# VITA-Group/FasterSeg

Hardware: NVIDIA H100
Metric: fasterseg_student_fps_1024x2048 (higher is better)
Workload: dtype fp16

## Files before the change

fasterseg_b200/csrc/conv_tc.cu:

```cuda
#include "fsb_common.cuh"
#include "fsb_internal.h"

namespace fsb {

constexpr int kTileM = 128;
constexpr int kMaxStages = 8;
constexpr int kThreads = 256;
constexpr int kAccLd = kTileM + 4;

struct ConvTcParams {
  CUtensorMap tmap_a[4];
  CUtensorMap tmap_b;
  CUtensorMap tmap_y[2];
  int tma_store;
  int tail_w;
  int taps;
  int tap_map[9];
  int tap_dh[9];
  int tap_dw[9];
  int tap_widx[9];
  int k_chunks;
  int Ho, Wo;
  int tiles_w, tiles_h;
  int tw, th;
  int win_pitch, win_rows;
  int win_sbo;
  int win_half;
  int win_stride;
  int m_half, m_grp;
  int Cout;
  int stages;
  int y_cstride;
  uint32_t flags;
  const float* scale;
  const float* shift;
  __half* y;
  float* stats;
  int stats_C;
  int stats_off;
};

template <int NT>
__host__ __device__ constexpr uint32_t conv_tc_out_bytes() { return static_cast<uint32_t>((NT + 63) / 64) * kTileM * 128; }
template <int NT>
__host__ __device__ constexpr uint32_t conv_tc_epilogue_bytes() { return conv_tc_out_bytes<NT>() + static_cast<uint32_t>(NT) * kAccLd * 4; }


template <int BK, int NT, bool WIN>
__global__ void __launch_bounds__(kThreads, NT <= 64 ? 2 : 1)
conv_tc_kernel(const __grid_constant__ ConvTcParams p) {
  extern __shared__ uint8_t smem_raw[];
  __shared__ __align__(8) uint64_t full_bar[kMaxStages];
  __shared__ __align__(8) uint64_t empty_bar[kMaxStages];
  __shared__ __align__(8) uint64_t win_full[2];
  __shared__ __align__(8) uint64_t win_empty[2];
  __shared__ float s_scale[NT];
  __shared__ float s_shift[NT];

  pdl_launch_dependents();
  const int warp = threadIdx.x >> 5;
  const int lane = threadIdx.x & 31;
  constexpr uint32_t kABytes = kTileM * BK * 2;
  constexpr uint32_t kStageBytes = WIN ? NT * BK * 2 : kABytes + NT * BK * 2;
  static_assert(!WIN || BK == 64, "windows are 128B-swizzled 64-channel rows");
  uint8_t* smem = reinterpret_cast<uint8_t*>((reinterpret_cast<uintptr_t>(smem_raw) + 1023) & ~uintptr_t(1023));

  int t = blockIdx.x;
  const int tile_w = t % p.tiles_w;
  t /= p.tiles_w;
  const int tile_h = t % p.tiles_h;
  const int img = t / p.tiles_h;
  const int w0 = tile_w * p.tw;
  const int h0 = tile_h * p.th;
  const int n0 = blockIdx.y * NT;
  const int k_iters = p.taps * p.k_chunks;

  if (warp == 0 && lane == 0) {
    tma_prefetch_desc(&p.tmap_a[0]);
    tma_prefetch_desc(&p.tmap_b);
    for (int s = 0; s < p.stages; ++s) {
      mbar_init(&full_bar[s], 1);
      mbar_init(&empty_bar[s], 4);
    }
    for (int w = 0; w < 2; ++w) {
      mbar_init(&win_full[w], 1);
      mbar_init(&win_empty[w], 4);
    }
    mbar_fence_init();
  }
  pdl_wait();
  for (int c = threadIdx.x; c < NT; c += kThreads) {
    const int ch = n0 + c;
    const bool ok = ch < p.Cout;
    s_scale[c] = (ok && (p.flags & FSB_CONV_AFFINE) && p.scale) ? p.scale[ch] : 1.0f;
    s_shift[c] = (ok && (p.flags & FSB_CONV_AFFINE) && p.shift) ? p.shift[ch] : 0.0f;
  }
  __syncthreads();

// ... 2 lines not shown
    const uint32_t win_bytes = static_cast<uint32_t>(p.win_rows * p.win_pitch) * 128u;
    RingPos rp, rw;
    for (int kc = 0; kc < p.k_chunks; ++kc) {
      mbar_wait_inline(&win_empty[rw.s], rw.phase ^ 1u);
      if (elect_one()) {
        mbar_arrive_expect_tx(&win_full[rw.s], win_bytes);
        tma_load_4d(smem + rw.s * p.win_stride, &p.tmap_a[0], &win_full[rw.s], kc * BK, w0 + p.tap_dw[0], h0 + p.tap_dh[0], img);
      }
      __syncwarp();
      rw.advance(2);
      for (int tap = 0; tap < 9; ++tap) {
        mbar_wait_inline(&empty_bar[rp.s], rp.phase ^ 1u);
        if (elect_one()) {
          mbar_arrive_expect_tx(&full_bar[rp.s], kStageBytes);
          tma_load_3d(bring + rp.s * kStageBytes, &p.tmap_b, &full_bar[rp.s], kc * BK, n0, tap);
        }
        __syncwarp();
        rp.advance(p.stages);
      }
    }
  } else if (warp == 0) {
    RingPos rp;
    uint8_t* sa = smem;
    for (int tap = 0; tap < p.taps; ++tap) {
      const CUtensorMap* ma = &p.tmap_a[p.tap_map[tap]];
      const int cw = w0 + p.tap_dw[tap];
      const int chh = h0 + p.tap_dh[tap];
      const int wi = p.tap_widx[tap];
      for (int kc = 0; kc < p.k_chunks; ++kc) {
        mbar_wait_inline(&empty_bar[rp.s], rp.phase ^ 1u);
        if (elect_one()) {
          mbar_arrive_expect_tx(&full_bar[rp.s], kStageBytes);
          tma_load_4d(sa, ma, &full_bar[rp.s], kc * BK, cw, chh, img);
          tma_load_3d(sa + kABytes, &p.tmap_b, &full_bar[rp.s], kc * BK, n0, wi);
        }
        __syncwarp();
        sa += kStageBytes;
        rp.advance(p.stages);
        if (rp.s == 0) sa = smem;
      }
    }
  } else if (warp >= 4) {
    const int tw = threadIdx.x - 128;
    float acc[2][NT / 2];
#pragma unroll
    for (int h = 0; h < 2; ++h)
#pragma unroll
      for (int i = 0; i < NT / 2; ++i) acc[h][i] = 0.f;
    const uint32_t sa0 = smem_u32(smem);
    const uint64_t da0 = wgmma_desc_kmajor(sa0, BK * 2);
    const uint64_t db0 = wgmma_desc_kmajor(sa0 + kABytes, BK * 2);
    constexpr uint32_t kHalf = (64 * BK * 2) >> 4;
    if constexpr (WIN) {
      const uint64_t dw0 = wgmma_desc(sa0, 16, p.win_sbo, 128);
      const uint64_t dbr = wgmma_desc_kmajor(sa0 + 2 * p.win_stride, 128);
      const uint64_t whalf = static_cast<uint64_t>(p.win_half * 8);
      RingPos rp, rw;
      int prev = -1, prev_w = -1;
      for (int kc = 0; kc < p.k_chunks; ++kc) {
        mbar_wait_inline(&win_full[rw.s], rw.phase);
        const uint64_t dwin = dw0 + static_cast<uint64_t>(rw.s * (p.win_stride >> 4));
        for (int tap = 0; tap < 9; ++tap) {
// ... 1 lines not shown
          mbar_wait_inline(&full_bar[rp.s], rp.phase);
          wgmma_fence();
          const uint64_t da = dwin + static_cast<uint64_t>((r * p.win_pitch + sx) * 8);
          const uint64_t db = dbr + static_cast<uint64_t>(rp.s * (kStageBytes >> 4));
#pragma unroll
          for (int k = 0; k < BK / 16; ++k) {
            wgmma_f16<NT, 0>(acc[0], da + static_cast<uint64_t>(2 * k), db + static_cast<uint64_t>(2 * k));
            wgmma_f16<NT, 0>(acc[1], da + whalf + static_cast<uint64_t>(2 * k), db + static_cast<uint64_t>(2 * k));
          }
          wgmma_commit();
          wgmma_wait<1>();
          if (prev >= 0 && lane == 0) mbar_arrive(&empty_bar[prev]);
          if (tap == 0 && prev_w >= 0 && lane == 0) mbar_arrive(&win_empty[prev_w]);
          prev = rp.s;
          rp.advance(p.stages);
        }
        prev_w = rw.s;
        rw.advance(2);
      }
    } else {
    RingPos rp;
    uint32_t doff = 0;
    int prev = -1;
    for (int it = 0; it < k_iters; ++it) {
      mbar_wait_inline(&full_bar[rp.s], rp.phase);
      wgmma_fence();
#pragma unroll
      for (int k = 0; k < BK / 16; ++k) {
        const uint64_t da = da0 + doff + static_cast<uint64_t>(2 * k), db = db0 + doff + static_cast<uint64_t>(2 * k);
        wgmma_f16<NT, 0>(acc[0], da, db);
        wgmma_f16<NT, 0>(acc[1], da + kHalf, db);
      }
      wgmma_commit();
      wgmma_wait<1>();
      if (prev >= 0 && lane == 0) mbar_arrive(&empty_bar[prev]);
      prev = rp.s;
      doff += kStageBytes >> 4;
      rp.advance(p.stages);
      if (rp.s == 0) doff = 0;
    }
    }
    wgmma_wait<0>();
    float* s_acc = reinterpret_cast<float*>(smem + conv_tc_out_bytes<NT>());
    named_bar_sync(1, 128);
    if constexpr (WIN) {
      const int row0 = wgmma_row(tw, 0);
      const int m0 = (row0 >> 3) * p.m_grp + (row0 & 7);
#pragma unroll
      for (int h = 0; h < 2; ++h) {
        float* s_h = s_acc + h * p.m_half + m0;
#pragma unroll
        for (int i = 0; i < NT / 2; ++i) s_h[wgmma_col(tw, i) * kAccLd + ((i >> 1) & 1) * p.m_grp] = acc[h][i];
      }
    } else {
#pragma unroll
      for (int h = 0; h < 2; ++h)
#pragma unroll
        for (int i = 0; i < NT / 2; ++i) s_acc[wgmma_col(tw, i) * kAccLd + 64 * h + wgmma_row(tw, i)] = acc[h][i];
    }
    named_bar_sync(1, 128);

    const int q = warp & 3;
    const int m = q * 32 + lane;
    const int oh = h0 + m / p.tw;
    const int ow = w0 + m % p.tw;
    const bool pix_ok = (oh < p.Ho) && (ow < p.Wo);
    __half* yrow = p.y + (static_cast<size_t>(img) * p.Ho * p.Wo + static_cast<size_t>(oh) * p.Wo + ow) * p.y_cstride + n0;
    const bool out_f32 = (p.flags & FSB_CONV_OUT_F32) != 0;
    float* yrow32 = reinterpret_cast<float*>(p.y) +
                    (static_cast<size_t>(img) * p.Ho * p.Wo + static_cast<size_t>(oh) * p.Wo + ow) * p.y_cstride + n0;
    const bool vec_ok = out_f32 ? ((reinterpret_cast<uintptr_t>(yrow32) & 15) == 0) : ((reinterpret_cast<uintptr_t>(yrow) & 15) == 0);
    const bool relu = (p.flags & FSB_CONV_RELU) != 0;
    const bool do_stats = (p.flags & FSB_CONV_STATS) != 0 && p.stats != nullptr;
    float* s_stat = reinterpret_cast<float*>(smem);
    for (int c0 = 0; c0 < NT; c0 += 64) {
      const int nb = min(4, (NT - c0) >> 4);
#pragma unroll
      for (int b = 0; b < 4; ++b) {
      if (b >= nb) break;
      const int c = c0 + 16 * b;
      float f[16];
#pragma unroll
      for (int j = 0; j < 16; ++j) f[j] = s_acc[(c + j) * kAccLd + m];
      if (do_stats) {
#pragma unroll
        for (int j = 0; j < 16; ++j) {
          float a = pix_ok ? f[j] : 0.f;
          float b = a * a;
#pragma unroll
          for (int o = 16; o > 0; o >>= 1) {
            a += __shfl_xor_sync(0xffffffffu, a, o);
            b += __shfl_xor_sync(0xffffffffu, b, o);
          }
          if (lane == 0) {
            s_stat[(q * 2 + 0) * NT + c + j] = a;
            s_stat[(q * 2 + 1) * NT + c + j] = b;
          }
        }
      }
#pragma unroll
      for (int j = 0; j < 16; ++j) {
        float x = f[j] * s_scale[c + j] + s_shift[c + j];
        f[j] = relu ? fmaxf(x, 0.f) : x;
      }
      if (pix_ok && out_f32) {
        const int remaining = p.Cout - (n0 + c);
        if (remaining >= 16 && vec_ok) {
          float4* dst = reinterpret_cast<float4*>(yrow32 + c);
          dst[0] = make_float4(f[0], f[1], f[2], f[3]);
          dst[1] = make_float4(f[4], f[5], f[6], f[7]);
          dst[2] = make_float4(f[8], f[9], f[10], f[11]);
          dst[3] = make_float4(f[12], f[13], f[14], f[15]);
        } else {
#pragma unroll
          for (int j = 0; j < 16; ++j)
            if (j < remaining) yrow32[c + j] = f[j];
        }
      } else if (p.tma_store) {
        uint4 o0, o1;
        o0.x = pack_half2(f[0], f[1]);
        o0.y = pack_half2(f[2], f[3]);
        o0.z = pack_half2(f[4], f[5]);
        o0.w = pack_half2(f[6], f[7]);
        o1.x = pack_half2(f[8], f[9]);
        o1.y = pack_half2(f[10], f[11]);
        o1.z = pack_half2(f[12], f[13]);
        o1.w = pack_half2(f[14], f[15]);
        uint8_t* slab = smem + static_cast<size_t>(c0 >> 6) * (kTileM * 128);
        const int ch16 = (c - c0) >> 3;
        if (NT - c0 >= 64) {
          *reinterpret_cast<uint4*>(slab + m * 128 + ((ch16 ^ (m & 7)) << 4)) = o0;
          *reinterpret_cast<uint4*>(slab + m * 128 + (((ch16 + 1) ^ (m & 7)) << 4)) = o1;
        } else {
          uint8_t* row = slab + m * (p.tail_w * 2) + (ch16 << 4);
          *reinterpret_cast<uint4*>(row) = o0;
          *reinterpret_cast<uint4*>(row + 16) = o1;
        }
      } else if (pix_ok) {
        const int remaining = p.Cout - (n0 + c);
        if (remaining >= 16 && vec_ok) {
          uint4 o0, o1;
          o0.x = pack_half2(f[0], f[1]);
          o0.y = pack_half2(f[2], f[3]);
          o0.z = pack_half2(f[4], f[5]);
          o0.w = pack_half2(f[6], f[7]);
          o1.x = pack_half2(f[8], f[9]);
          o1.y = pack_half2(f[10], f[11]);
          o1.z = pack_half2(f[12], f[13]);
          o1.w = pack_half2(f[14], f[15]);
          uint4* dst = reinterpret_cast<uint4*>(yrow + c);
          dst[0] = o0;
          dst[1] = o1;
        } else {
#pragma unroll
          for (int j = 0; j < 16; ++j)
            if (j < remaining) yrow[c + j] = __float2half_rn(f[j]);
        }
      }
      }
      if (p.tma_store) {
        fence_proxy_async_smem();
        named_bar_sync(1, 128);
        if (warp == 4 && lane == 0) {
          const bool full = (NT - c0) >= 64;
          tma_store_4d(&p.tmap_y[full ? 0 : 1], smem + static_cast<size_t>(c0 >> 6) * (kTileM * 128), n0 + c0, w0, h0, img);
          tma_store_commit();
        }
      }
    }
    if (p.tma_store && warp == 4 && lane == 0) tma_store_wait_read();
    if (do_stats) {
      named_bar_sync(2, 128);
      float* row = p.stats + static_cast<size_t>(blockIdx.x) * 2 * p.stats_C + p.stats_off;
      for (int ch = static_cast<int>(threadIdx.x) - 128; ch < NT; ch += 128) {
        if (n0 + ch >= p.Cout) continue;
        float a = s_stat[0 * NT + ch], b = s_stat[1 * NT + ch];
#pragma unroll
        for (int w = 1; w < 4; ++w) {
          a += s_stat[(w * 2 + 0) * NT + ch];
          b += s_stat[(w * 2 + 1) * NT + ch];
        }
        row[n0 + ch] = a;
        row[p.stats_C + n0 + ch] = b;
      }
    }
  }
  __syncthreads();
}

static int encode_tiled(CUtensorMap* map, const void* base, int rank, const uint64_t* dims, const uint64_t* strides_bytes,
                        const uint32_t* box, int swizzle_bytes) {
  PFN_encodeTiled enc = get_encode_tiled();
  if (!enc) return set_error(FSB_ERR_CUDA, "cuTensorMapEncodeTiled entry point unavailable");
  cuuint32_t estr[5] = {1, 1, 1, 1, 1};
  cuuint64_t gdim[5];
  cuuint64_t gstr[5];
  cuuint32_t bdim[5];
  for (int i = 0; i < rank; ++i) {
    gdim[i] = dims[i];
    bdim[i] = box[i];
  }
  for (int i = 0; i + 1 < rank; ++i) gstr[i] = strides_bytes[i];
  CUtensorMapSwizzle sw = swizzle_bytes == 128 ? CU_TENSOR_MAP_SWIZZLE_128B
                          : (swizzle_bytes == 64 ? CU_TENSOR_MAP_SWIZZLE_64B
                                                 : (swizzle_bytes == 32 ? CU_TENSOR_MAP_SWIZZLE_32B : CU_TENSOR_MAP_SWIZZLE_NONE));
  CUresult r = enc(map, CU_TENSOR_MAP_DATA_TYPE_FLOAT16, static_cast<cuuint32_t>(rank), const_cast<void*>(base), gdim, gstr,
                   bdim, estr, CU_TENSOR_MAP_INTERLEAVE_NONE, sw, CU_TENSOR_MAP_L2_PROMOTION_L2_256B,
                   CU_TENSOR_MAP_FLOAT_OOB_FILL_NONE);
  if (r != CUDA_SUCCESS) {
    char buf[256];
// ... 25 lines not shown

enum ConvTcMode { kPerTap, kWindow, kStrip };
static ConvTcMode conv_tc_mode(const fsb_conv_desc* d) {
  if (d->ksize != 3 || d->stride != 1 || d->dil != 1) return kPerTap;
  const int o = opt(OPT_CONV_TC2);
  if (o == 0) return kPerTap;
  if (o == 2 && d->Cin % 64 == 0 && !(d->flags & FSB_CONV_STATS)) return kStrip;
  return kWindow;
}
bool conv_tc_strip(const fsb_conv_desc* d) { return conv_tc_mode(d) == kStrip; }

int conv_tc_m_tiles(const fsb_conv_desc* d) {
  if (conv_tc_strip(d)) return ((d->Wo + kTileM - 1) / kTileM) * d->Ho * d->N;
  const int tw = d->Wo >= 16 ? 16 : 8, th = kTileM / tw;
  return ((d->Wo + tw - 1) / tw) * ((d->Ho + th - 1) / th) * d->N;
}

int conv_tc_supported(const fsb_conv_desc* d) {
  if (d->Cin < 16 || (d->x_cstride % 8) != 0) return 0;
  if (!(d->ksize == 1 || d->ksize == 3) || !(d->stride == 1 || d->stride == 2)) return 0;
  return 1;
}

template <int BK, int NT, bool WIN = false>
static int conv_tc_run(dim3 grid, size_t smem_bytes, cudaStream_t stream, const ConvTcParams& p) {
  if (int rc = ensure_dyn_smem(reinterpret_cast<const void*>(conv_tc_kernel<BK, NT, WIN>), 220 * 1024, "cudaFuncSetAttribute(conv_tc)"))
    return rc;
  const cudaError_t e = launch_kernel(conv_tc_kernel<BK, NT, WIN>, grid, dim3(kThreads), smem_bytes, stream, p);
  return e == cudaSuccess ? FSB_OK : set_cuda_error(e, "conv_tc launch");
}

template <int BK, bool WIN>
static int conv_tc_run_nt(int n_tile, dim3 grid, size_t smem_bytes, cudaStream_t stream, const ConvTcParams& p) {
  switch (n_tile) {
    case 16: return conv_tc_run<BK, 16, WIN>(grid, smem_bytes, stream, p);
    case 32: return conv_tc_run<BK, 32, WIN>(grid, smem_bytes, stream, p);
    case 48: return conv_tc_run<BK, 48, WIN>(grid, smem_bytes, stream, p);
    case 64: return conv_tc_run<BK, 64, WIN>(grid, smem_bytes, stream, p);
    case 96: return conv_tc_run<BK, 96, WIN>(grid, smem_bytes, stream, p);
    default: return conv_tc_run<BK, 128, WIN>(grid, smem_bytes, stream, p);
  }
}

int conv_tc_launch(const fsb_conv_desc* d, const void* x, const void* wpacked, const float* scale, const float* shift,
                   void* y, float* stats, cudaStream_t stream, const ConvTcCustom* cu, bool window_ok) {
  const ConvGeom g = conv_geom(d);
  if (cu && (d->stride != 1 || (d->flags & (FSB_CONV_OUT_F32 | FSB_CONV_STATS))))
    return set_error(FSB_ERR_INVALID, "conv_tc: custom tap tables need a stride-1 fp16 problem");
  if ((reinterpret_cast<uintptr_t>(x) & 15) || (reinterpret_cast<uintptr_t>(wpacked) & 15))
    return set_error(FSB_ERR_INVALID, "conv_tc: x / wpacked must be 16-byte aligned");
  ConvTcParams p;
  memset(&p, 0, sizeof(p));
  const ConvTcMode mode = cu ? kPerTap : conv_tc_mode(d);
  const bool strip = mode == kStrip;
  p.taps = cu ? cu->ntaps : g.taps;
  p.Ho = cu ? cu->Ho : d->Ho;
  p.Wo = cu ? cu->Wo : d->Wo;
  p.tw = strip ? kTileM : (p.Wo >= 16 ? 16 : 8);
  p.th = kTileM / p.tw;
  p.tiles_w = (p.Wo + p.tw - 1) / p.tw;
  p.tiles_h = (p.Ho + p.th - 1) / p.th;
  for (int i = 0; i < 9; ++i) p.tap_widx[i] = i;
  p.Cout = d->Cout;
  static const int kNt[] = {16, 32, 48, 64, 96, 128};
  const int m_tiles = p.tiles_w * p.tiles_h * d->N;
  int n_tiles = (g.npad + 127) / 128;
  int ni = 0;
  while (kNt[ni] * n_tiles < g.npad) ++ni;
  int n_tile = kNt[ni];
  n_tiles = (g.npad + n_tile - 1) / n_tile;
  const int sms = sm_count();
  const int nt_min = opt(OPT_CONV_NTILE_MIN) >= 16 ? opt(OPT_CONV_NTILE_MIN) : 32;
  while (m_tiles * n_tiles < sms && ni > 0 && kNt[ni - 1] >= nt_min) {
    n_tile = kNt[--ni];
    n_tiles = (g.npad + n_tile - 1) / n_tile;
  }
  const bool win = strip || (mode == kWindow && ((window_ok && m_tiles * n_tiles > sms && !(d->flags & FSB_CONV_STATS)) ||
                                                 opt(OPT_CONV_TC2) == 1));
  const int bk = win ? 64 : g.bk;
  p.k_chunks = (g.kpad + bk - 1) / bk;
  if (win) {
    p.win_pitch = p.tw + 2;
    p.win_rows = p.th + 2;
    p.win_stride = (p.win_rows * p.win_pitch * 128 + 1023) / 1024 * 1024;
    p.m_half = 64;
    p.m_grp = 8;
    if (strip) {
      p.win_sbo = 8 * 128;
      p.win_half = 64;
    } else if (p.tw == 16) {
      p.win_sbo = p.win_pitch * 128;
      p.win_half = 8;
      p.m_half = 8;
      p.m_grp = 16;
    } else {
      p.win_sbo = p.win_pitch * 128;
      p.win_half = 8 * p.win_pitch;
    }
  }
  p.y_cstride = d->y_cstride;
  p.flags = d->flags;
  p.scale = scale;
  p.shift = shift;
  p.y = static_cast<__half*>(y);
  p.stats = stats;
  p.stats_C = d->stats_C > 0 ? d->stats_C : d->Cout;
  p.stats_off = d->stats_off;
  if ((d->flags & FSB_CONV_STATS) && stats && (d->stats_off < 0 || d->stats_off + d->Cout > p.stats_C))
    return set_error(FSB_ERR_INVALID, "conv_tc: stats_off + Cout exceeds stats_C");

  const size_t stage_bytes = (win ? 0 : static_cast<size_t>(kTileM) * bk * 2) + static_cast<size_t>(n_tile) * bk * 2;
  const int k_iters = p.taps * p.k_chunks;
  const size_t smem_budget = (n_tile == 128 || m_tiles * n_tiles <= sms || strip) ? 200 * 1024 : 100 * 1024;
  const size_t win_bytes = win ? 2 * static_cast<size_t>(p.win_stride) : 0;
  int stages = static_cast<int>((smem_budget - win_bytes) / stage_bytes);
  if (stages < 2) stages = 2;
  if (stages > kMaxStages) stages = kMaxStages;
  if (stages > k_iters) stages = k_iters;
  p.stages = stages;
  const size_t epi_bytes = n_tile == 16 ? conv_tc_epilogue_bytes<16>() : n_tile == 32 ? conv_tc_epilogue_bytes<32>()
                           : n_tile == 48 ? conv_tc_epilogue_bytes<48>() : n_tile == 64 ? conv_tc_epilogue_bytes<64>()
                           : n_tile == 96 ? conv_tc_epilogue_bytes<96>() : conv_tc_epilogue_bytes<128>();
  size_t smem_bytes = (win_bytes + stage_bytes * stages > epi_bytes ? win_bytes + stage_bytes * stages : epi_bytes) + 1024;
  p.tma_store = 0;
  if (!(d->flags & (FSB_CONV_OUT_F32 | FSB_CONV_STATS)) && d->Cout % 8 == 0 && d->y_cstride % 8 == 0 && (reinterpret_cast<uintptr_t>(y) & 15) == 0 &&
      n_tile % 8 == 0 && (cu || opt(OPT_NO_TMA_STORE) <= 0)) {
    const uint64_t ycs = static_cast<uint64_t>(d->y_cstride) * 2;
    uint64_t dims[4] = {static_cast<uint64_t>(d->Cout), static_cast<uint64_t>(d->Wo), static_cast<uint64_t>(d->Ho),
                        static_cast<uint64_t>(d->N)};
    uint64_t str[3] = {ycs, ycs * d->Wo, ycs * d->Wo * d->Ho};
    if (cu) {
      y = const_cast<void*>(cu->y_base);
      for (int i = 0; i < 4; ++i) dims[i] = cu->y_dims[i];
      for (int i = 0; i < 3; ++i) str[i] = cu->y_strides[i];
    }
    const uint32_t box64[4] = {64u, static_cast<uint32_t>(p.tw), static_cast<uint32_t>(p.th), 1u};
    int rc = 0;
    if (n_tile >= 64) rc = encode_tiled(&p.tmap_y[0], y, 4, dims, str, box64, 128);
    p.tail_w = n_tile % 64;
    if (!rc && p.tail_w) {
      const uint32_t boxt[4] = {static_cast<uint32_t>(p.tail_w), static_cast<uint32_t>(p.tw), static_cast<uint32_t>(p.th), 1u};
      rc = encode_tiled(&p.tmap_y[1], y, 4, dims, str, boxt, 0);
    }
    if (rc) return rc;
    if (n_tile < 64) p.tmap_y[0] = p.tmap_y[1];
    p.tma_store = 1;
  }
  if (cu && !p.tma_store) return set_error(FSB_ERR_UNSUPPORTED, "conv_tc: custom output lattice needs the TMA-store epilogue");
// ... 36 lines not shown
        used[ph * 2 + pw] = true;
      }
    for (int ph = 0; ph < 2; ++ph)
      for (int pw = 0; pw < 2; ++pw) {
        if (!used[ph * 2 + pw]) continue;
        const int Hp = (d->H - ph + 1) / 2, Wp = (d->W - pw + 1) / 2;
        if (Hp <= 0 || Wp <= 0) return set_error(FSB_ERR_INVALID, "conv_tc: empty parity plane");
        const uint64_t dims[4] = {static_cast<uint64_t>(d->Cin), static_cast<uint64_t>(Wp), static_cast<uint64_t>(Hp),
                                  static_cast<uint64_t>(d->N)};
        const uint64_t str[3] = {2 * cs, 2 * cs * d->W, cs * d->W * d->H};
        const __half* base = xb + (static_cast<size_t>(ph) * d->W + pw) * d->x_cstride;
        int rc = encode_tiled(&p.tmap_a[ph * 2 + pw], base, 4, dims, str, boxA, g.bk * 2);
        if (rc) return rc;
      }
    if (!used[0]) p.tmap_a[0] = p.tmap_a[p.tap_map[0]];
  }
  {
    const uint64_t dims[3] = {static_cast<uint64_t>(g.kpad), static_cast<uint64_t>(g.npad), static_cast<uint64_t>(g.taps)};
    const uint64_t str[2] = {static_cast<uint64_t>(g.kpad) * 2, static_cast<uint64_t>(g.kpad) * g.npad * 2};
    const uint32_t boxB[3] = {static_cast<uint32_t>(bk), static_cast<uint32_t>(n_tile), 1u};
    int rc = encode_tiled(&p.tmap_b, wpacked, 3, dims, str, boxB, bk * 2);
    if (rc) return rc;
  }
  const dim3 grid(static_cast<unsigned>(m_tiles), static_cast<unsigned>(n_tiles));
  if (win) return conv_tc_run_nt<64, true>(n_tile, grid, smem_bytes, stream, p);
  if (g.bk == 64) return conv_tc_run_nt<64, false>(n_tile, grid, smem_bytes, stream, p);
  return conv_tc_run_nt<32, false>(n_tile, grid, smem_bytes, stream, p);
}

}
```

fasterseg_b200/csrc/fsb_common.cuh:

```cuda
#pragma once
#include <cuda.h>
#include <cuda_fp16.h>
#include <cuda_runtime.h>
#include <stdint.h>
#include <stdio.h>

namespace fsb {

__device__ __forceinline__ uint32_t smem_u32(const void* p) {
  return static_cast<uint32_t>(__cvta_generic_to_shared(p));
}
__device__ __forceinline__ bool elect_one() {
  uint32_t pred = 0;
  asm volatile(
      "{\n\t.reg .pred P;\n\telect.sync _|P, 0xffffffff;\n\tselp.u32 %0, 1, 0, P;\n\t}\n"
      : "=r"(pred));
  return pred != 0;
}

__device__ __forceinline__ void pdl_launch_dependents() { asm volatile("griddepcontrol.launch_dependents;" ::: "memory"); }
__device__ __forceinline__ void pdl_wait() { asm volatile("griddepcontrol.wait;" ::: "memory"); }

__device__ __forceinline__ void mbar_init(uint64_t* bar, uint32_t count) {
  asm volatile("mbarrier.init.shared::cta.b64 [%0], %1;" ::"r"(smem_u32(bar)), "r"(count) : "memory");
// ... 73 lines not shown
__device__ __forceinline__ void tma_store_4d(const CUtensorMap* m, const void* smem_src, int c0, int c1, int c2, int c3) {
  asm volatile("cp.async.bulk.tensor.4d.global.shared::cta.bulk_group [%0, {%2, %3, %4, %5}], [%1];"
               ::"l"(reinterpret_cast<uint64_t>(m)), "r"(smem_u32(smem_src)), "r"(c0), "r"(c1), "r"(c2), "r"(c3)
               : "memory");
}
__device__ __forceinline__ void tma_store_commit() { asm volatile("cp.async.bulk.commit_group;" ::: "memory"); }
__device__ __forceinline__ void tma_store_wait_read() { asm volatile("cp.async.bulk.wait_group.read 0;" ::: "memory"); }
__device__ __forceinline__ void fence_proxy_async_smem() { asm volatile("fence.proxy.async.shared::cta;" ::: "memory"); }
__device__ __forceinline__ void named_bar_sync(int id, int nthreads) {
  asm volatile("bar.sync %0, %1;" ::"r"(id), "r"(nthreads) : "memory");
}

__device__ __forceinline__ void cluster_sync_all_threads() {
  asm volatile("barrier.cluster.arrive.release.aligned;\n\tbarrier.cluster.wait.acquire.aligned;" ::: "memory");
}
__device__ __forceinline__ uint32_t mapa_cluster(uint32_t cta_smem_addr, uint32_t target_rank) {
  uint32_t r;
  asm volatile("mapa.shared::cluster.u32 %0, %1, %2;" : "=r"(r) : "r"(cta_smem_addr), "r"(target_rank));
  return r;
}
__device__ __forceinline__ void st_cluster_u32(uint32_t cluster_addr, uint32_t v) {
  asm volatile("st.shared::cluster.u32 [%0], %1;" ::"r"(cluster_addr), "r"(v) : "memory");
}

__device__ __forceinline__ void wgmma_fence() { asm volatile("wgmma.fence.sync.aligned;" ::: "memory"); }
__device__ __forceinline__ void wgmma_commit() { asm volatile("wgmma.commit_group.sync.aligned;" ::: "memory"); }
template <int N>
__device__ __forceinline__ void wgmma_wait() { asm volatile("wgmma.wait_group.sync.aligned %0;" ::"n"(N) : "memory"); }
__device__ __forceinline__ int wgmma_row(int t, int i) { return 16 * (t >> 5) + ((t & 31) >> 2) + 8 * ((i >> 1) & 1); }
__device__ __forceinline__ int wgmma_col(int t, int i) { return 8 * (i >> 2) + 2 * (t & 3) + (i & 1); }

template <int TR>
__device__ __forceinline__ void wgmma_m64n16k16(float (&d)[8], uint64_t da, uint64_t db) {
  asm volatile(
      "wgmma.mma_async.sync.aligned.m64n16k16.f32.f16.f16 "
      "{%0, %1, %2, %3, %4, %5, %6, %7}, %8, %9, 1, 1, 1, %10, %11;"
      : "+f"(d[0]), "+f"(d[1]), "+f"(d[2]), "+f"(d[3]), "+f"(d[4]), "+f"(d[5]), "+f"(d[6]), "+f"(d[7])
      : "l"(da), "l"(db), "n"(TR), "n"(TR));
}
template <int TR>
__device__ __forceinline__ void wgmma_m64n32k16(float (&d)[16], uint64_t da, uint64_t db) {
  asm volatile(
      "wgmma.mma_async.sync.aligned.m64n32k16.f32.f16.f16 "
      "{%0, %1, %2, %3, %4, %5, %6, %7, %8, %9, %10, %11, %12, %13, %14, %15}, %16, %17, 1, 1, 1, %18, %19;"
      : "+f"(d[0]), "+f"(d[1]), "+f"(d[2]), "+f"(d[3]), "+f"(d[4]), "+f"(d[5]), "+f"(d[6]), "+f"(d[7]), "+f"(d[8]), "+f"(d[9]), "+f"(d[10]), "+f"(d[11]), "+f"(d[12]), "+f"(d[13]), "+f"(d[14]), "+f"(d[15])
      : "l"(da), "l"(db), "n"(TR), "n"(TR));
// ... 65 lines not shown
```

fasterseg_b200/csrc/fsb_internal.h:

```cpp
#pragma once
#include <cuda.h>
#include <cuda_runtime.h>
#include <stdint.h>
#include <stdio.h>
#include <stdlib.h>
#include <string.h>

#include "../../include/fsb200.h"

namespace fsb {

int set_error(int code, const char* msg);
int set_cuda_error(cudaError_t e, const char* where);

typedef CUresult (*PFN_encodeTiled)(CUtensorMap*, CUtensorMapDataType, cuuint32_t, void*, const cuuint64_t*,
                                    const cuuint64_t*, const cuuint32_t*, const cuuint32_t*, CUtensorMapInterleave,
                                    CUtensorMapSwizzle, CUtensorMapL2promotion, CUtensorMapFloatOOBfill);
PFN_encodeTiled get_encode_tiled();

struct ConvGeom {
  int taps;
  int bk;
  int kpad;
  int npad;
// ... 7 lines not shown
  OPT_CONV_TC2 = 0,
  OPT_TC2_R,
  OPT_TC2_ASTAGES,
  OPT_NO_TMA_STORE,
  OPT_DGRAD_S2_DIRECT,
  OPT_WGRAD_TC,
  OPT_CONV_PERSIST,
  OPT_PERSIST_OCC,
  OPT_PERSIST_STAGES,
  OPT_UPSAMPLE_V2,
  OPT_DETERMINISTIC,
  OPT_CONV_TC3,
  OPT_CONV_TC4,
  OPT_CONV_TC5,
  OPT_CONV_KSPLIT,
  OPT_CONV_NTILE_MIN,
  OPT_COUNT
};
int opt(Opt o);

int ensure_dyn_smem(const void* kernel, int bytes, const char* what);

template <typename... KArgs, typename... Args>
inline cudaError_t launch_kernel(void (*kernel)(KArgs...), dim3 grid, dim3 block, size_t smem, cudaStream_t stream,
                                 Args&&... args) {
  cudaLaunchConfig_t cfg;
  memset(&cfg, 0, sizeof(cfg));
  cfg.gridDim = grid;
  cfg.blockDim = block;
  cfg.dynamicSmemBytes = smem;
  cfg.stream = stream;
  cudaLaunchAttribute attr[1];
  attr[0].id = cudaLaunchAttributeProgrammaticStreamSerialization;
  attr[0].val.programmaticStreamSerializationAllowed = 1;
  cfg.attrs = attr;
  cfg.numAttrs = pdl_enabled() ? 1 : 0;
  return cudaLaunchKernelEx(&cfg, kernel, static_cast<KArgs>(args)...);
}

extern thread_local cudaError_t g_launch_err;
#define FSB_LAUNCH(kernel, grid, block, smem, stream, ...) \
  (::fsb::g_launch_err = ::fsb::launch_kernel(kernel, grid, block, smem, stream, __VA_ARGS__))
inline cudaError_t last_launch_error() {
  cudaError_t e = g_launch_err;
  g_launch_err = cudaSuccess;
  if (e == cudaSuccess) e = cudaGetLastError();
  return e;
}

struct ConvTcCustom {
  int ntaps;
  int dh[9], dw[9], widx[9];
  int Ho, Wo;
  const void* y_base;
  uint64_t y_dims[4];
  uint64_t y_strides[3];
};
int conv_tc_supported(const fsb_conv_desc* d);
bool conv_tc_strip(const fsb_conv_desc* d);
int conv_tc_launch(const fsb_conv_desc* d, const void* x, const void* wpacked, const float* scale, const float* shift,
                   void* y, float* stats, cudaStream_t stream, const ConvTcCustom* cu = nullptr, bool window_ok = true);
int conv_wgrad_tc_supported(const fsb_conv_desc* d, int dy_cstride);
int conv_wgrad_tc_launch(const fsb_conv_desc* d, const void* x, const void* dy, int dcs, float* dw, int64_t so, int64_t si,
                         float gscale, cudaStream_t stream);
int conv_direct_launch(const fsb_conv_desc* d, const void* x, const void* wpacked, const float* scale, const float* shift,
// ... 4 lines not shown
```

fasterseg_b200/csrc/wgrad_tc.cu:

```cuda
#include "fsb_common.cuh"
#include "fsb_internal.h"

namespace fsb {

constexpr int kWgThreads = 256;
constexpr int kWgMaxStages = 6;
constexpr int kWgPix = 128;
constexpr int kWgSub = kWgPix * 128;

struct WgradTcParams {
  CUtensorMap tmap_dy;
  CUtensorMap tmap_x[4];
  int taps, ksize;
  int tap_map[9], tap_dh[9], tap_dw[9];
  int tiles_w, tiles_h, n_img;
  int tw, th;
  int Cout, Cin;
  int co_tiles, ci_tiles;
  int chunks;
  int stages;
  float inv_gscale;
  float* dw;
  long long so, si;
};
// ... 191 lines not shown
        const int ph = ((qh % 2) + 2) % 2, pw = ((qw % 2) + 2) % 2;
        p.tap_map[tp] = ph * 2 + pw;
        p.tap_dh[tp] = floordiv2(qh);
        p.tap_dw[tp] = floordiv2(qw);
        used[ph * 2 + pw] = true;
      }
    for (int ph = 0; ph < 2; ++ph)
      for (int pw = 0; pw < 2; ++pw) {
        if (!used[ph * 2 + pw]) continue;
        const int Hp = (d->H - ph + 1) / 2, Wp = (d->W - pw + 1) / 2;
        if (Hp <= 0 || Wp <= 0) return set_error(FSB_ERR_INVALID, "wgrad_tc: empty parity plane");
        const uint64_t dims[4] = {static_cast<uint64_t>(d->Cin), static_cast<uint64_t>(Wp), static_cast<uint64_t>(Hp),
                                  static_cast<uint64_t>(d->N)};
        const uint64_t str[3] = {2 * cs, 2 * cs * d->W, cs * d->W * d->H};
        int rc = encode_tiled_generic(&p.tmap_x[ph * 2 + pw], xb + (static_cast<size_t>(ph) * d->W + pw) * d->x_cstride, 4, dims,
                                      str, box, 128);
        if (rc) return rc;
      }
  }
  const void* kernel = ci_tile == 128 ? reinterpret_cast<const void*>(conv_wgrad_tc_kernel<128>)
                                      : reinterpret_cast<const void*>(conv_wgrad_tc_kernel<64>);
  if (int rc = ensure_dyn_smem(kernel, 220 * 1024, "cudaFuncSetAttribute(conv_wgrad_tc)")) return rc;
  dim3 grid(static_cast<unsigned>(fixed), static_cast<unsigned>(chunks));
  const cudaError_t e = ci_tile == 128 ? launch_kernel(conv_wgrad_tc_kernel<128>, grid, dim3(kWgThreads), smem_bytes, stream, p)
                                       : launch_kernel(conv_wgrad_tc_kernel<64>, grid, dim3(kWgThreads), smem_bytes, stream, p);
  if (e != cudaSuccess) return set_cuda_error(e, "conv_wgrad_tc launch");
  return FSB_OK;
}

}
```

Baseline: 2136.

## Add cluster-based split-K for tensor-core conv with DSMEM reduction

```diff
diff --git a/fasterseg_b200/csrc/conv_tc.cu b/fasterseg_b200/csrc/conv_tc.cu
--- a/fasterseg_b200/csrc/conv_tc.cu
+++ b/fasterseg_b200/csrc/conv_tc.cu
@@ -46,7 +46,7 @@
 __host__ __device__ constexpr uint32_t conv_tc_epilogue_bytes() { return conv_tc_out_bytes<NT>() + static_cast<uint32_t>(NT) * kAccLd * 4; }
 
 
-template <int BK, int NT, bool WIN>
+template <int BK, int NT, bool WIN, bool SPLIT>
 __global__ void __launch_bounds__(kThreads, NT <= 64 ? 2 : 1)
 conv_tc_kernel(const __grid_constant__ ConvTcParams p) {
   extern __shared__ uint8_t smem_raw[];
@@ -63,6 +63,7 @@
   constexpr uint32_t kABytes = kTileM * BK * 2;
   constexpr uint32_t kStageBytes = WIN ? NT * BK * 2 : kABytes + NT * BK * 2;
   static_assert(!WIN || BK == 64, "windows are 128B-swizzled 64-channel rows");
+  static_assert(!(WIN && SPLIT), "the K split runs on the per-tap mode only");
   uint8_t* smem = reinterpret_cast<uint8_t*>((reinterpret_cast<uintptr_t>(smem_raw) + 1023) & ~uintptr_t(1023));
 
   int t = blockIdx.x;
@@ -74,6 +75,8 @@
   const int h0 = tile_h * p.th;
   const int n0 = blockIdx.y * NT;
   const int k_iters = p.taps * p.k_chunks;
+  const int it_begin = SPLIT ? static_cast<int>(blockIdx.z) * k_iters / static_cast<int>(gridDim.z) : 0;
+  const int it_end = SPLIT ? static_cast<int>(blockIdx.z + 1) * k_iters / static_cast<int>(gridDim.z) : k_iters;
 
   if (warp == 0 && lane == 0) {
     tma_prefetch_desc(&p.tmap_a[0]);
@@ -122,22 +125,21 @@
   } else if (warp == 0) {
     RingPos rp;
     uint8_t* sa = smem;
-    for (int tap = 0; tap < p.taps; ++tap) {
-      const CUtensorMap* ma = &p.tmap_a[p.tap_map[tap]];
-      const int cw = w0 + p.tap_dw[tap];
-      const int chh = h0 + p.tap_dh[tap];
-      const int wi = p.tap_widx[tap];
-      for (int kc = 0; kc < p.k_chunks; ++kc) {
-        mbar_wait_inline(&empty_bar[rp.s], rp.phase ^ 1u);
-        if (elect_one()) {
-          mbar_arrive_expect_tx(&full_bar[rp.s], kStageBytes);
-          tma_load_4d(sa, ma, &full_bar[rp.s], kc * BK, cw, chh, img);
-          tma_load_3d(sa + kABytes, &p.tmap_b, &full_bar[rp.s], kc * BK, n0, wi);
-        }
-        __syncwarp();
-        sa += kStageBytes;
-        rp.advance(p.stages);
-        if (rp.s == 0) sa = smem;
+    int tap = it_begin / p.k_chunks, kc = it_begin - tap * p.k_chunks;
+    for (int it = it_begin; it < it_end; ++it) {
+      mbar_wait_inline(&empty_bar[rp.s], rp.phase ^ 1u);
+      if (elect_one()) {
+        mbar_arrive_expect_tx(&full_bar[rp.s], kStageBytes);
+        tma_load_4d(sa, &p.tmap_a[p.tap_map[tap]], &full_bar[rp.s], kc * BK, w0 + p.tap_dw[tap], h0 + p.tap_dh[tap], img);
+        tma_load_3d(sa + kABytes, &p.tmap_b, &full_bar[rp.s], kc * BK, n0, p.tap_widx[tap]);
+      }
+      __syncwarp();
+      sa += kStageBytes;
+      rp.advance(p.stages);
+      if (rp.s == 0) sa = smem;
+      if (++kc == p.k_chunks) {
+        kc = 0;
+        ++tap;
       }
     }
   } else if (warp >= 4) {
@@ -185,7 +187,7 @@
     RingPos rp;
     uint32_t doff = 0;
     int prev = -1;
-    for (int it = 0; it < k_iters; ++it) {
+    for (int it = it_begin; it < it_end; ++it) {
       mbar_wait_inline(&full_bar[rp.s], rp.phase);
       wgmma_fence();
 #pragma unroll
@@ -223,85 +225,64 @@
     }
     named_bar_sync(1, 128);
 
-    const int q = warp & 3;
-    const int m = q * 32 + lane;
-    const int oh = h0 + m / p.tw;
-    const int ow = w0 + m % p.tw;
-    const bool pix_ok = (oh < p.Ho) && (ow < p.Wo);
-    __half* yrow = p.y + (static_cast<size_t>(img) * p.Ho * p.Wo + static_cast<size_t>(oh) * p.Wo + ow) * p.y_cstride + n0;
-    const bool out_f32 = (p.flags & FSB_CONV_OUT_F32) != 0;
-    float* yrow32 = reinterpret_cast<float*>(p.y) +
-                    (static_cast<size_t>(img) * p.Ho * p.Wo + static_cast<size_t>(oh) * p.Wo + ow) * p.y_cstride + n0;
-    const bool vec_ok = out_f32 ? ((reinterpret_cast<uintptr_t>(yrow32) & 15) == 0) : ((reinterpret_cast<uintptr_t>(yrow) & 15) == 0);
-    const bool relu = (p.flags & FSB_CONV_RELU) != 0;
-    const bool do_stats = (p.flags & FSB_CONV_STATS) != 0 && p.stats != nullptr;
-    float* s_stat = reinterpret_cast<float*>(smem);
-    for (int c0 = 0; c0 < NT; c0 += 64) {
-      const int nb = min(4, (NT - c0) >> 4);
-#pragma unroll
-      for (int b = 0; b < 4; ++b) {
-      if (b >= nb) break;
-      const int c = c0 + 16 * b;
-      float f[16];
-#pragma unroll
-      for (int j = 0; j < 16; ++j) f[j] = s_acc[(c + j) * kAccLd + m];
-      if (do_stats) {
+    if constexpr (!SPLIT) {
+      const int q = warp & 3;
+      const int m = q * 32 + lane;
+      const int oh = h0 + m / p.tw;
+      const int ow = w0 + m % p.tw;
+      const bool pix_ok = (oh < p.Ho) && (ow < p.Wo);
+      __half* yrow = p.y + (static_cast<size_t>(img) * p.Ho * p.Wo + static_cast<size_t>(oh) * p.Wo + ow) * p.y_cstride + n0;
+      const bool out_f32 = (p.flags & FSB_CONV_OUT_F32) != 0;
+      float* yrow32 = reinterpret_cast<float*>(p.y) +
+                      (static_cast<size_t>(img) * p.Ho * p.Wo + static_cast<size_t>(oh) * p.Wo + ow) * p.y_cstride + n0;
+      const bool vec_ok = out_f32 ? ((reinterpret_cast<uintptr_t>(yrow32) & 15) == 0) : ((reinterpret_cast<uintptr_t>(yrow) & 15) == 0);
+      const bool relu = (p.flags & FSB_CONV_RELU) != 0;
+      const bool do_stats = (p.flags & FSB_CONV_STATS) != 0 && p.stats != nullptr;
+      float* s_stat = reinterpret_cast<float*>(smem);
+      for (int c0 = 0; c0 < NT; c0 += 64) {
+        const int nb = min(4, (NT - c0) >> 4);
+#pragma unroll
+        for (int b = 0; b < 4; ++b) {
+        if (b >= nb) break;
+        const int c = c0 + 16 * b;
+        float f[16];
+#pragma unroll
+        for (int j = 0; j < 16; ++j) f[j] = s_acc[(c + j) * kAccLd + m];
+        if (do_stats) {
+#pragma unroll
+          for (int j = 0; j < 16; ++j) {
+            float a = pix_ok ? f[j] : 0.f;
+            float b = a * a;
+#pragma unroll
+            for (int o = 16; o > 0; o >>= 1) {
+              a += __shfl_xor_sync(0xffffffffu, a, o);
+              b += __shfl_xor_sync(0xffffffffu, b, o);
+            }
+            if (lane == 0) {
+              s_stat[(q * 2 + 0) * NT + c + j] = a;
+              s_stat[(q * 2 + 1) * NT + c + j] = b;
+            }
+          }
+        }
 #pragma unroll
         for (int j = 0; j < 16; ++j) {
-          float a = pix_ok ? f[j] : 0.f;
-          float b = a * a;
-#pragma unroll
-          for (int o = 16; o > 0; o >>= 1) {
-            a += __shfl_xor_sync(0xffffffffu, a, o);
-            b += __shfl_xor_sync(0xffffffffu, b, o);
-          }
-          if (lane == 0) {
-            s_stat[(q * 2 + 0) * NT + c + j] = a;
-            s_stat[(q * 2 + 1) * NT + c + j] = b;
-          }
-        }
-      }
-#pragma unroll
-      for (int j = 0; j < 16; ++j) {
-        float x = f[j] * s_scale[c + j] + s_shift[c + j];
-        f[j] = relu ? fmaxf(x, 0.f) : x;
-      }
-      if (pix_ok && out_f32) {
-        const int remaining = p.Cout - (n0 + c);
-        if (remaining >= 16 && vec_ok) {
-          float4* dst = reinterpret_cast<float4*>(yrow32 + c);
-          dst[0] = make_float4(f[0], f[1], f[2], f[3]);
-          dst[1] = make_float4(f[4], f[5], f[6], f[7]);
-          dst[2] = make_float4(f[8], f[9], f[10], f[11]);
-          dst[3] = make_float4(f[12], f[13], f[14], f[15]);
-        } else {
-#pragma unroll
-          for (int j = 0; j < 16; ++j)
-            if (j < remaining) yrow32[c + j] = f[j];
-        }
-      } else if (p.tma_store) {
-        uint4 o0, o1;
-        o0.x = pack_half2(f[0], f[1]);
-        o0.y = pack_half2(f[2], f[3]);
-        o0.z = pack_half2(f[4], f[5]);
-        o0.w = pack_half2(f[6], f[7]);
-        o1.x = pack_half2(f[8], f[9]);
-        o1.y = pack_half2(f[10], f[11]);
-        o1.z = pack_half2(f[12], f[13]);
-        o1.w = pack_half2(f[14], f[15]);
-        uint8_t* slab = smem + static_cast<size_t>(c0 >> 6) * (kTileM * 128);
-        const int ch16 = (c - c0) >> 3;
-        if (NT - c0 >= 64) {
-          *reinterpret_cast<uint4*>(slab + m * 128 + ((ch16 ^ (m & 7)) << 4)) = o0;
-          *reinterpret_cast<uint4*>(slab + m * 128 + (((ch16 + 1) ^ (m & 7)) << 4)) = o1;
-        } else {
-          uint8_t* row = slab + m * (p.tail_w * 2) + (ch16 << 4);
-          *reinterpret_cast<uint4*>(row) = o0;
-          *reinterpret_cast<uint4*>(row + 16) = o1;
-        }
-      } else if (pix_ok) {
-        const int remaining = p.Cout - (n0 + c);
-        if (remaining >= 16 && vec_ok) {
+          float x = f[j] * s_scale[c + j] + s_shift[c + j];
+          f[j] = relu ? fmaxf(x, 0.f) : x;
+        }
+        if (pix_ok && out_f32) {
+          const int remaining = p.Cout - (n0 + c);
+          if (remaining >= 16 && vec_ok) {
+            float4* dst = reinterpret_cast<float4*>(yrow32 + c);
+            dst[0] = make_float4(f[0], f[1], f[2], f[3]);
+            dst[1] = make_float4(f[4], f[5], f[6], f[7]);
+            dst[2] = make_float4(f[8], f[9], f[10], f[11]);
+            dst[3] = make_float4(f[12], f[13], f[14], f[15]);
+          } else {
+#pragma unroll
+            for (int j = 0; j < 16; ++j)
+              if (j < remaining) yrow32[c + j] = f[j];
+          }
+        } else if (p.tma_store) {
           uint4 o0, o1;
           o0.x = pack_half2(f[0], f[1]);
           o0.y = pack_half2(f[2], f[3]);
@@ -311,44 +292,120 @@
           o1.y = pack_half2(f[10], f[11]);
           o1.z = pack_half2(f[12], f[13]);
           o1.w = pack_half2(f[14], f[15]);
-          uint4* dst = reinterpret_cast<uint4*>(yrow + c);
-          dst[0] = o0;
-          dst[1] = o1;
+          uint8_t* slab = smem + static_cast<size_t>(c0 >> 6) * (kTileM * 128);
+          const int ch16 = (c - c0) >> 3;
+          if (NT - c0 >= 64) {
+            *reinterpret_cast<uint4*>(slab + m * 128 + ((ch16 ^ (m & 7)) << 4)) = o0;
+            *reinterpret_cast<uint4*>(slab + m * 128 + (((ch16 + 1) ^ (m & 7)) << 4)) = o1;
+          } else {
+            uint8_t* row = slab + m * (p.tail_w * 2) + (ch16 << 4);
+            *reinterpret_cast<uint4*>(row) = o0;
+            *reinterpret_cast<uint4*>(row + 16) = o1;
+          }
+        } else if (pix_ok) {
+          const int remaining = p.Cout - (n0 + c);
+          if (remaining >= 16 && vec_ok) {
+            uint4 o0, o1;
+            o0.x = pack_half2(f[0], f[1]);
+            o0.y = pack_half2(f[2], f[3]);
+            o0.z = pack_half2(f[4], f[5]);
+            o0.w = pack_half2(f[6], f[7]);
+            o1.x = pack_half2(f[8], f[9]);
+            o1.y = pack_half2(f[10], f[11]);
+            o1.z = pack_half2(f[12], f[13]);
+            o1.w = pack_half2(f[14], f[15]);
+            uint4* dst = reinterpret_cast<uint4*>(yrow + c);
+            dst[0] = o0;
+            dst[1] = o1;
+          } else {
+#pragma unroll
+            for (int j = 0; j < 16; ++j)
+              if (j < remaining) yrow[c + j] = __float2half_rn(f[j]);
+          }
+        }
+        }
+        if (p.tma_store) {
+          fence_proxy_async_smem();
+          named_bar_sync(1, 128);
+          if (warp == 4 && lane == 0) {
+            const bool full = (NT - c0) >= 64;
+            tma_store_4d(&p.tmap_y[full ? 0 : 1], smem + static_cast<size_t>(c0 >> 6) * (kTileM * 128), n0 + c0, w0, h0, img);
+            tma_store_commit();
+          }
+        }
+      }
+      if (p.tma_store && warp == 4 && lane == 0) tma_store_wait_read();
+      if (do_stats) {
+        named_bar_sync(2, 128);
+        float* row = p.stats + static_cast<size_t>(blockIdx.x) * 2 * p.stats_C + p.stats_off;
+        for (int ch = static_cast<int>(threadIdx.x) - 128; ch < NT; ch += 128) {
+          if (n0 + ch >= p.Cout) continue;
+          float a = s_stat[0 * NT + ch], b = s_stat[1 * NT + ch];
+#pragma unroll
+          for (int w = 1; w < 4; ++w) {
+            a += s_stat[(w * 2 + 0) * NT + ch];
+            b += s_stat[(w * 2 + 1) * NT + ch];
+          }
+          row[n0 + ch] = a;
+          row[p.stats_C + n0 + ch] = b;
+        }
+      }
+    }
+  }
+  if constexpr (SPLIT) {
+    cluster_sync_all_threads();
+    const int S = static_cast<int>(gridDim.z), z = static_cast<int>(blockIdx.z);
+    const int q0 = z * (kTileM / 4) / S, nq = (z + 1) * (kTileM / 4) / S - q0;
+    const uint32_t acc_addr = smem_u32(smem + conv_tc_out_bytes<NT>());
+    const bool relu = (p.flags & FSB_CONV_RELU) != 0;
+    for (int item = threadIdx.x; item < nq * (NT / 8); item += kThreads) {
+      const int m = 4 * (q0 + item % nq);
+      const int c = 8 * (item / nq);
+      float4 v[8];
+      for (int r = 0; r < S; ++r) {
+        float4 t[8];
+#pragma unroll
+        for (int j = 0; j < 8; ++j) t[j] = ld_cluster_f32x4(mapa_cluster(acc_addr + ((c + j) * kAccLd + m) * 4, r));
+#pragma unroll
+        for (int j = 0; j < 8; ++j) {
+          if (r == 0) {
+            v[j] = t[j];
+          } else {
+            v[j].x += t[j].x;
+            v[j].y += t[j].y;
+            v[j].z += t[j].z;
+            v[j].w += t[j].w;
+          }
+        }
+      }
+      const int remaining = p.Cout - (n0 + c);
+#pragma unroll
+      for (int i = 0; i < 4; ++i) {
+        const int oh = h0 + (m + i) / p.tw;
+        const int ow = w0 + (m + i) % p.tw;
+        if (oh >= p.Ho || ow >= p.Wo || remaining <= 0) continue;
+        float f[8];
+#pragma unroll
+        for (int j = 0; j < 8; ++j) {
+          const float a = i == 0 ? v[j].x : i == 1 ? v[j].y : i == 2 ? v[j].z : v[j].w;
+          const float x = a * s_scale[c + j] + s_shift[c + j];
+          f[j] = relu ? fmaxf(x, 0.f) : x;
+        }
+        __half* dst = p.y + (static_cast<size_t>(img) * p.Ho * p.Wo + static_cast<size_t>(oh) * p.Wo + ow) * p.y_cstride + n0 + c;
+        if (remaining >= 8 && (reinterpret_cast<uintptr_t>(dst) & 15) == 0) {
+          *reinterpret_cast<uint4*>(dst) = make_uint4(pack_half2(f[0], f[1]), pack_half2(f[2], f[3]), pack_half2(f[4], f[5]),
+                                                      pack_half2(f[6], f[7]));
         } else {
 #pragma unroll
-          for (int j = 0; j < 16; ++j)
-            if (j < remaining) yrow[c + j] = __float2half_rn(f[j]);
-        }
-      }
-      }
-      if (p.tma_store) {
-        fence_proxy_async_smem();
-        named_bar_sync(1, 128);
-        if (warp == 4 && lane == 0) {
-          const bool full = (NT - c0) >= 64;
-          tma_store_4d(&p.tmap_y[full ? 0 : 1], smem + static_cast<size_t>(c0 >> 6) * (kTileM * 128), n0 + c0, w0, h0, img);
-          tma_store_commit();
-        }
-      }
-    }
-    if (p.tma_store && warp == 4 && lane == 0) tma_store_wait_read();
-    if (do_stats) {
-      named_bar_sync(2, 128);
-      float* row = p.stats + static_cast<size_t>(blockIdx.x) * 2 * p.stats_C + p.stats_off;
-      for (int ch = static_cast<int>(threadIdx.x) - 128; ch < NT; ch += 128) {
-        if (n0 + ch >= p.Cout) continue;
-        float a = s_stat[0 * NT + ch], b = s_stat[1 * NT + ch];
-#pragma unroll
-        for (int w = 1; w < 4; ++w) {
-          a += s_stat[(w * 2 + 0) * NT + ch];
-          b += s_stat[(w * 2 + 1) * NT + ch];
-        }
-        row[n0 + ch] = a;
-        row[p.stats_C + n0 + ch] = b;
-      }
-    }
-  }
-  __syncthreads();
+          for (int j = 0; j < 8; ++j)
+            if (j < remaining) dst[j] = __float2half_rn(f[j]);
+        }
+      }
+    }
+    cluster_sync_all_threads();
+  } else {
+    __syncthreads();
+  }
 }
 
 static int encode_tiled(CUtensorMap* map, const void* base, int rank, const uint64_t* dims, const uint64_t* strides_bytes,
@@ -420,23 +477,24 @@
   return 1;
 }
 
-template <int BK, int NT, bool WIN = false>
+template <int BK, int NT, bool WIN, bool SPLIT>
 static int conv_tc_run(dim3 grid, size_t smem_bytes, cudaStream_t stream, const ConvTcParams& p) {
-  if (int rc = ensure_dyn_smem(reinterpret_cast<const void*>(conv_tc_kernel<BK, NT, WIN>), 220 * 1024, "cudaFuncSetAttribute(conv_tc)"))
+  if (int rc = ensure_dyn_smem(reinterpret_cast<const void*>(conv_tc_kernel<BK, NT, WIN, SPLIT>), 220 * 1024,
+                               "cudaFuncSetAttribute(conv_tc)"))
     return rc;
-  const cudaError_t e = launch_kernel(conv_tc_kernel<BK, NT, WIN>, grid, dim3(kThreads), smem_bytes, stream, p);
+  const cudaError_t e = launch_kernel(grid.z, conv_tc_kernel<BK, NT, WIN, SPLIT>, grid, dim3(kThreads), smem_bytes, stream, p);
   return e == cudaSuccess ? FSB_OK : set_cuda_error(e, "conv_tc launch");
 }
 
-template <int BK, bool WIN>
+template <int BK, bool WIN, bool SPLIT = false>
 static int conv_tc_run_nt(int n_tile, dim3 grid, size_t smem_bytes, cudaStream_t stream, const ConvTcParams& p) {
   switch (n_tile) {
-    case 16: return conv_tc_run<BK, 16, WIN>(grid, smem_bytes, stream, p);
-    case 32: return conv_tc_run<BK, 32, WIN>(grid, smem_bytes, stream, p);
-    case 48: return conv_tc_run<BK, 48, WIN>(grid, smem_bytes, stream, p);
-    case 64: return conv_tc_run<BK, 64, WIN>(grid, smem_bytes, stream, p);
-    case 96: return conv_tc_run<BK, 96, WIN>(grid, smem_bytes, stream, p);
-    default: return conv_tc_run<BK, 128, WIN>(grid, smem_bytes, stream, p);
+    case 16: return conv_tc_run<BK, 16, WIN, SPLIT>(grid, smem_bytes, stream, p);
+    case 32: return conv_tc_run<BK, 32, WIN, SPLIT>(grid, smem_bytes, stream, p);
+    case 48: return conv_tc_run<BK, 48, WIN, SPLIT>(grid, smem_bytes, stream, p);
+    case 64: return conv_tc_run<BK, 64, WIN, SPLIT>(grid, smem_bytes, stream, p);
+    case 96: return conv_tc_run<BK, 96, WIN, SPLIT>(grid, smem_bytes, stream, p);
+    default: return conv_tc_run<BK, 128, WIN, SPLIT>(grid, smem_bytes, stream, p);
   }
 }
 
@@ -477,6 +535,18 @@
                                                  opt(OPT_CONV_TC2) == 1));
   const int bk = win ? 64 : g.bk;
   p.k_chunks = (g.kpad + bk - 1) / bk;
+  const int k_iters = p.taps * p.k_chunks;
+  int split = 1;
+  const int ksplit = opt(OPT_CONV_KSPLIT);
+  if (ksplit >= 2 && !cu && !win && window_ok && !(d->flags & (FSB_CONV_OUT_F32 | FSB_CONV_STATS))) {
+    split = ksplit < 8 ? ksplit : 8;
+    if (split > k_iters) split = k_iters;
+    n_tiles = (g.npad + 127) / 128;
+    ni = 0;
+    while (kNt[ni] * n_tiles < g.npad) ++ni;
+    n_tile = kNt[ni];
+    n_tiles = (g.npad + n_tile - 1) / n_tile;
+  }
   if (win) {
     p.win_pitch = p.tw + 2;
     p.win_rows = p.th + 2;
@@ -508,20 +578,20 @@
     return set_error(FSB_ERR_INVALID, "conv_tc: stats_off + Cout exceeds stats_C");
 
   const size_t stage_bytes = (win ? 0 : static_cast<size_t>(kTileM) * bk * 2) + static_cast<size_t>(n_tile) * bk * 2;
-  const int k_iters = p.taps * p.k_chunks;
-  const size_t smem_budget = (n_tile == 128 || m_tiles * n_tiles <= sms || strip) ? 200 * 1024 : 100 * 1024;
+  const size_t smem_budget = (n_tile == 128 || m_tiles * n_tiles * split <= sms || strip) ? 200 * 1024 : 100 * 1024;
   const size_t win_bytes = win ? 2 * static_cast<size_t>(p.win_stride) : 0;
   int stages = static_cast<int>((smem_budget - win_bytes) / stage_bytes);
   if (stages < 2) stages = 2;
   if (stages > kMaxStages) stages = kMaxStages;
-  if (stages > k_iters) stages = k_iters;
+  const int rank_iters = (k_iters + split - 1) / split;
+  if (stages > rank_iters) stages = rank_iters;
   p.stages = stages;
   const size_t epi_bytes = n_tile == 16 ? conv_tc_epilogue_bytes<16>() : n_tile == 32 ? conv_tc_epilogue_bytes<32>()
                            : n_tile == 48 ? conv_tc_epilogue_bytes<48>() : n_tile == 64 ? conv_tc_epilogue_bytes<64>()
                            : n_tile == 96 ? conv_tc_epilogue_bytes<96>() : conv_tc_epilogue_bytes<128>();
   size_t smem_bytes = (win_bytes + stage_bytes * stages > epi_bytes ? win_bytes + stage_bytes * stages : epi_bytes) + 1024;
   p.tma_store = 0;
-  if (!(d->flags & (FSB_CONV_OUT_F32 | FSB_CONV_STATS)) && d->Cout % 8 == 0 && d->y_cstride % 8 == 0 && (reinterpret_cast<uintptr_t>(y) & 15) == 0 &&
+  if (split == 1 && !(d->flags & (FSB_CONV_OUT_F32 | FSB_CONV_STATS)) && d->Cout % 8 == 0 && d->y_cstride % 8 == 0 && (reinterpret_cast<uintptr_t>(y) & 15) == 0 &&
       n_tile % 8 == 0 && (cu || opt(OPT_NO_TMA_STORE) <= 0)) {
     const uint64_t ycs = static_cast<uint64_t>(d->y_cstride) * 2;
     uint64_t dims[4] = {static_cast<uint64_t>(d->Cout), static_cast<uint64_t>(d->Wo), static_cast<uint64_t>(d->Ho),
@@ -604,7 +674,10 @@
     int rc = encode_tiled(&p.tmap_b, wpacked, 3, dims, str, boxB, bk * 2);
     if (rc) return rc;
   }
-  const dim3 grid(static_cast<unsigned>(m_tiles), static_cast<unsigned>(n_tiles));
+  const dim3 grid(static_cast<unsigned>(m_tiles), static_cast<unsigned>(n_tiles), static_cast<unsigned>(split));
+  if (split > 1)
+    return g.bk == 64 ? conv_tc_run_nt<64, false, true>(n_tile, grid, smem_bytes, stream, p)
+                      : conv_tc_run_nt<32, false, true>(n_tile, grid, smem_bytes, stream, p);
   if (win) return conv_tc_run_nt<64, true>(n_tile, grid, smem_bytes, stream, p);
   if (g.bk == 64) return conv_tc_run_nt<64, false>(n_tile, grid, smem_bytes, stream, p);
   return conv_tc_run_nt<32, false>(n_tile, grid, smem_bytes, stream, p);
diff --git a/fasterseg_b200/csrc/fsb_common.cuh b/fasterseg_b200/csrc/fsb_common.cuh
--- a/fasterseg_b200/csrc/fsb_common.cuh
+++ b/fasterseg_b200/csrc/fsb_common.cuh
@@ -119,6 +119,12 @@
 __device__ __forceinline__ void st_cluster_u32(uint32_t cluster_addr, uint32_t v) {
   asm volatile("st.shared::cluster.u32 [%0], %1;" ::"r"(cluster_addr), "r"(v) : "memory");
 }
+__device__ __forceinline__ float4 ld_cluster_f32x4(uint32_t cluster_addr) {
+  float4 v;
+  asm volatile("ld.shared::cluster.v4.f32 {%0, %1, %2, %3}, [%4];"
+               : "=f"(v.x), "=f"(v.y), "=f"(v.z), "=f"(v.w) : "r"(cluster_addr) : "memory");
+  return v;
+}
 
 __device__ __forceinline__ void wgmma_fence() { asm volatile("wgmma.fence.sync.aligned;" ::: "memory"); }
 __device__ __forceinline__ void wgmma_commit() { asm volatile("wgmma.commit_group.sync.aligned;" ::: "memory"); }
diff --git a/fasterseg_b200/csrc/fsb_internal.h b/fasterseg_b200/csrc/fsb_internal.h
--- a/fasterseg_b200/csrc/fsb_internal.h
+++ b/fasterseg_b200/csrc/fsb_internal.h
@@ -53,25 +53,33 @@
 int ensure_dyn_smem(const void* kernel, int bytes, const char* what);
 
 template <typename... KArgs, typename... Args>
-inline cudaError_t launch_kernel(void (*kernel)(KArgs...), dim3 grid, dim3 block, size_t smem, cudaStream_t stream,
-                                 Args&&... args) {
+inline cudaError_t launch_kernel(unsigned cluster_z, void (*kernel)(KArgs...), dim3 grid, dim3 block, size_t smem,
+                                 cudaStream_t stream, Args&&... args) {
   cudaLaunchConfig_t cfg;
   memset(&cfg, 0, sizeof(cfg));
   cfg.gridDim = grid;
   cfg.blockDim = block;
   cfg.dynamicSmemBytes = smem;
   cfg.stream = stream;
-  cudaLaunchAttribute attr[1];
-  attr[0].id = cudaLaunchAttributeProgrammaticStreamSerialization;
-  attr[0].val.programmaticStreamSerializationAllowed = 1;
+  cudaLaunchAttribute attr[2];
+  int n = 0;
+  if (pdl_enabled()) {
+    attr[n].id = cudaLaunchAttributeProgrammaticStreamSerialization;
+    attr[n++].val.programmaticStreamSerializationAllowed = 1;
+  }
+  if (cluster_z > 1) {
+    attr[n].id = cudaLaunchAttributeClusterDimension;
+    attr[n].val.clusterDim.x = 1;
+    attr[n].val.clusterDim.y = 1;
+    attr[n++].val.clusterDim.z = cluster_z;
+  }
   cfg.attrs = attr;
-  cfg.numAttrs = pdl_enabled() ? 1 : 0;
+  cfg.numAttrs = n;
   return cudaLaunchKernelEx(&cfg, kernel, static_cast<KArgs>(args)...);
 }
 
 extern thread_local cudaError_t g_launch_err;
-#define FSB_LAUNCH(kernel, grid, block, smem, stream, ...) \
-  (::fsb::g_launch_err = ::fsb::launch_kernel(kernel, grid, block, smem, stream, __VA_ARGS__))
+#define FSB_LAUNCH(...) (::fsb::g_launch_err = ::fsb::launch_kernel(1u, __VA_ARGS__))
 inline cudaError_t last_launch_error() {
   cudaError_t e = g_launch_err;
   g_launch_err = cudaSuccess;
diff --git a/fasterseg_b200/csrc/wgrad_tc.cu b/fasterseg_b200/csrc/wgrad_tc.cu
--- a/fasterseg_b200/csrc/wgrad_tc.cu
+++ b/fasterseg_b200/csrc/wgrad_tc.cu
@@ -237,8 +237,8 @@
                                       : reinterpret_cast<const void*>(conv_wgrad_tc_kernel<64>);
   if (int rc = ensure_dyn_smem(kernel, 220 * 1024, "cudaFuncSetAttribute(conv_wgrad_tc)")) return rc;
   dim3 grid(static_cast<unsigned>(fixed), static_cast<unsigned>(chunks));
-  const cudaError_t e = ci_tile == 128 ? launch_kernel(conv_wgrad_tc_kernel<128>, grid, dim3(kWgThreads), smem_bytes, stream, p)
-                                       : launch_kernel(conv_wgrad_tc_kernel<64>, grid, dim3(kWgThreads), smem_bytes, stream, p);
+  const cudaError_t e = ci_tile == 128 ? launch_kernel(1u, conv_wgrad_tc_kernel<128>, grid, dim3(kWgThreads), smem_bytes, stream, p)
+                                       : launch_kernel(1u, conv_wgrad_tc_kernel<64>, grid, dim3(kWgThreads), smem_bytes, stream, p);
   if (e != cudaSuccess) return set_cuda_error(e, "conv_wgrad_tc launch");
   return FSB_OK;
 }
```

New measurement: 2176 (median of 6 runs). 1.9% higher.
